# Kateridge/TransMF_AD

Hardware: AMD Instinct MI355X
Metric: volume-pairs/sec fwd+bwd(+Adam), 96^3 MRI+PET batch=8 per GPU (higher is better)
Workload: dtype f32

## Files before the change

transmf_ad_amd/csrc/conv1_gram.hip:

```cpp
#include "tmf_common.h"

namespace {

constexpr int GT_D = 8, GT_H = 8, GT_W = 32;
constexpr int GP_D = GT_D + 2, GP_H = GT_H + 4, GP_W = GT_W + 4;
constexpr int GTHR = 512, GWG = 256, NACC = 64;

__host__ __device__ constexpr int kidx(int dd, int dh, int dw) {
    return dd == 0 ? (dh == 0 ? dw : 3 + (dh - 1) * 5 + (dw + 2)) : 13 + ((dd - 1) * 5 + (dh + 2)) * 5 + (dw + 2);
}
static_assert(kidx(2, 2, 2) == 62, "63 offsets");

typedef double f64x2 __attribute__((ext_vector_type(2)));
__device__ __forceinline__ float rbf16(float v) { return __builtin_bit_cast(float, tmf_pack_bf16(v, 0.f) << 16); }

__global__ __launch_bounds__(GTHR) void c1_gram_kernel(const float* __restrict__ x, double* __restrict__ part,
                                                        int D, int H, int W, int tilesD, int tilesH, int tilesW, int ntiles, int round16) {
    constexpr int NT = GP_D * GP_H * GP_W, NS = NT > 8 * GTHR ? NT : 8 * GTHR;
    __shared__ __attribute__((aligned(16))) double smem[NS];
    double* tile = smem;
    double* red = smem;
    const int tid = threadIdx.x;
    const int g = tid & 7, hh = (tid >> 3) & 7, dd0 = tid >> 6;
    double acc[63];
// ... 62 lines not shown
    }
    const int lane = tid & 63, kq = tid >> 6;
#pragma unroll
    for (int c = 0; c < 8; ++c) {
        __syncthreads();
#pragma unroll
        for (int q = 0; q < 8; ++q) {
            const int k = c * 8 + q;
            red[q * GTHR + tid] = k < 63 ? acc[k < 63 ? k : 0] : ssum;
        }
        __syncthreads();
        double s = 0.0;
#pragma unroll
        for (int m = 0; m < 8; ++m) s += red[kq * GTHR + m * 64 + lane];
#pragma unroll
        for (int o = 32; o > 0; o >>= 1) s += __shfl_xor(s, o);
        if (lane == 0) part[(size_t)blockIdx.x * NACC + c * 8 + kq] = s;
    }
}

constexpr int GMAXC = 64;

constexpr int NGRAM = 760;
constexpr int HWG = 64, HTHR = 256, HNB = 288, HPART = 96;
constexpr int HNE = (HNB * 9 + HTHR - 1) / HTHR;

__host__ __device__ constexpr int class_tap(int cls, int j) {
    const int ax = cls >> 1, fixed = (cls & 1) ? 0 : 2, a = j / 3, b = j % 3;
    return ax == 0 ? fixed * 9 + a * 3 + b : (ax == 1 ? a * 9 + fixed * 3 + b : a * 9 + b * 3 + fixed);
}

__global__ __launch_bounds__(HTHR) void c1_shell_gram_kernel(const float* __restrict__ x, double* __restrict__ part, int B, int D, int H, int W,
                                                              int round16) {
    __shared__ double xs[HNB * 9];
    __shared__ int vbase[HNB], vcrd[HNB];
    __shared__ double red[3 * 81];
    const int tid = threadIdx.x, cls = blockIdx.y, ax = cls >> 1, side = cls & 1;
    const int n1 = ax == 0 ? H + 2 : D, n2 = ax == 2 ? H : W + 2;
    const int per = n1 * n2, total = B * per;
    const int p = tid % 81, slice = tid / 81, pi = p / 9, pj = p % 9;
    int cv_[HNE], cdd[HNE], cdh[HNE], cdw[HNE];
#pragma unroll
    for (int k = 0; k < HNE; ++k) {
        const int e = tid + k * HTHR, vi = e / 9, j = e - vi * 9, tap = class_tap(cls, j);
        cv_[k] = e < HNB * 9 ? vi : -1;
        cdd[k] = tap / 9 - 2; cdh[k] = (tap / 3) % 3 - 2; cdw[k] = tap % 3 - 2;
    }
    double acc = 0.0, eacc = 0.0;
    for (int base = blockIdx.x * HNB; base < total; base += gridDim.x * HNB) {
        __syncthreads();
        for (int vt = tid; vt < HNB; vt += HTHR) {
            const int s_ = base + vt;
            int c = -1, off = 0;
            if (s_ < total) {
                const int b = s_ / per, q = s_ - b * per, q1 = q / n2, q2 = q - q1 * n2;
                int vd, vh, vw;
                if (ax == 0) { vd = side ? D : -1; vh = q1 - 1; vw = q2 - 1; }
                else if (ax == 1) { vh = side ? H : -1; vd = q1; vw = q2 - 1; }
                else { vw = side ? W : -1; vd = q1; vh = q2; }
                c = (vd + 1) | (vh + 1) << 10 | (vw + 1) << 20;
                off = b * D * H * W;
            }
            vcrd[vt] = c; vbase[vt] = off;
        }
        __syncthreads();
#pragma unroll
        for (int k = 0; k < HNE; ++k) {
            if (cv_[k] < 0) continue;
            const int c = vcrd[cv_[k]];
            float v = 0.f;
            if (c >= 0) {
                const int ud = (c & 1023) + cdd[k], uh = ((c >> 10) & 1023) + cdh[k], uw = (c >> 20) + cdw[k];
                if (ud >= 0 && ud < D && uh >= 0 && uh < H && uw >= 0 && uw < W) v = x[(size_t)vbase[cv_[k]] + ((size_t)ud * H + uh) * W + uw];
            }
            xs[tid + k * HTHR] = (double)(round16 ? rbf16(v) : v);
        }
        __syncthreads();
        if (slice < 3) {
#pragma unroll 8
            for (int vi = slice * (HNB / 3); vi < (slice + 1) * (HNB / 3); ++vi) {
                const double xa = xs[vi * 9 + pi];
                acc = fma(xa, xs[vi * 9 + pj], acc);
                eacc += pj == 0 ? xa : 0.0;
            }
        }
    }
    __shared__ double rede[3 * 9];
    __syncthreads();
    if (slice < 3) {
        red[slice * 81 + p] = acc;
        if (pj == 0) rede[slice * 9 + pi] = eacc;
    }
    __syncthreads();
    double* row = part + ((size_t)cls * gridDim.x + blockIdx.x) * HPART;
    if (tid < 81) row[tid] = (red[tid] + red[81 + tid]) + red[162 + tid];
    else if (tid < 90) row[tid] = (rede[tid - 81] + rede[9 + tid - 81]) + rede[18 + tid - 81];
}

__global__ __launch_bounds__(1024) void c1_gram2_finish_kernel(const float* __restrict__ w, const double* __restrict__ rpart, int ngram,
                                                                const double* __restrict__ hpart, int nh, double* __restrict__ gram,
                                                                float* __restrict__ out, int C, int round16) {
    __shared__ double ra[16 * NACC];
    __shared__ double R[NACC];
    __shared__ double Hc[6 * HPART];
    __shared__ double G[27 * 27 + 27];
    __shared__ float wsh[27 * GMAXC];
    __shared__ double rows[27 * GMAXC];
    const int tid = threadIdx.x;
    {
        const int k = tid & 63, rg = tid >> 6;
        double s = 0.0;
#pragma unroll 8
        for (int i = rg; i < ngram; i += 16) s += rpart[(size_t)i * NACC + k];
        ra[rg * NACC + k] = s;
    }
    for (int e = tid; e < 27 * C; e += 1024) wsh[e] = round16 ? rbf16(w[e]) : w[e];
    for (int e = tid; e < 6 * HPART; e += 1024) {
        const int cls = e / HPART, k = e - cls * HPART;
        double s0 = 0.0, s1_ = 0.0, s2_ = 0.0, s3 = 0.0;
// ... 155 lines not shown
```

transmf_ad_amd/csrc/conv3d_mfma.hip:

```cpp
#include <type_traits>
#include "tmf_device.h"

#ifndef TMF_CONV_ACC
#define TMF_CONV_ACC 1
#endif
#ifndef TMF_CONV_BUF
#define TMF_CONV_BUF 1
#endif

namespace {

template <int KS_, int CINC_, int MT_, int NT_, int WM_, int WN_, int TD_, int TH_, int TW_, int TPS_>
struct FwdCfg {
    static constexpr int KS = KS_, CINC = CINC_, MT = MT_, NT = NT_, WM = WM_, WN = WN_;
    static constexpr int TD = TD_, TH = TH_, TW = TW_, TPS = TPS_;
    static constexpr int PAD = KS / 2;
    static constexpr int HD = TD + 2 * PAD, HH = TH + 2 * PAD, HW = TW + 2 * PAD;
    static constexpr int NHALO = HD * HH * HW;
    static constexpr int CP = CINC + 4;
    static constexpr int NPOS = TD * TH * TW;
    static constexpr int NB = 32 * NT * WN;
    static constexpr int NTAPS = KS * KS * KS;
    static constexpr int NSTAGES = NTAPS / TPS;
    static constexpr int BSTAGE = TPS * CINC * NB;
// ... 1111 lines not shown
        else mma_bricks(std::integral_constant<int, 3>{});
    }

#pragma unroll
    for (int t = 0; t < C::TPW; ++t) {
        const int tap0 = C::PACK ? 2 * (wave + 8 * t) : tap_base + t;
        if (t < tap_cnt && tap0 < 27) {
#pragma unroll
            for (int j = 0; j < C::NT; ++j) {
                const int co = co0 + j * 32 + l31;
#pragma unroll
                for (int r = 0; r < 16; ++r) {
                    const int m = (r & 3) + 8 * (r >> 2) + 4 * hsel;
                    const int tap = C::PACK ? tap0 + (r >> 3) : tap0;
                    const int ci = ci0 + (C::PACK ? (m & 15) : m);
                    if (tap < 27 && ci < Cin && co < Cout)
                        partial[(((size_t)split * 27 + tap) * Cin + ci) * Cout + co] = acc[t][j][r];
                }
            }
        }
    }
}

template <int NT>
__global__ __launch_bounds__(256) void conv1x1_wgrad_kernel(
    const float* __restrict__ x, const float* __restrict__ dz, float* __restrict__ partial,
    long npos, int Cin, int Cout, int slabs_per_block) {
    const int tid = threadIdx.x;
    const int lane = tid & 63;
    const int wave = __builtin_amdgcn_readfirstlane(tid >> 6);
    const int l31 = lane & 31, hsel = lane >> 5;
    const int ci = blockIdx.y * 32 + l31;
    const int co0 = blockIdx.z * 32 * NT;
    f32x16 acc[NT];
#pragma unroll
    for (int j = 0; j < NT; ++j)
#pragma unroll
        for (int r = 0; r < 16; ++r) acc[j][r] = 0.f;
    const long p_begin = ((long)blockIdx.x * slabs_per_block) * 256 + wave * 64;
    for (int sl = 0; sl < slabs_per_block; ++sl) {
        const long pb = p_begin + (long)sl * 256;
#pragma unroll 8
        for (int q = 0; q < 32; ++q) {
            const long p = pb + 2 * q + hsel;
            const bool pv = p < npos;
            const float av = (pv && ci < Cin) ? x[p * Cin + ci] : 0.f;
#pragma unroll
            for (int j = 0; j < NT; ++j) {
                const int co = co0 + j * 32 + l31;
                const float bv = (pv && co < Cout) ? dz[p * Cout + co] : 0.f;
                acc[j] = __builtin_amdgcn_mfma_f32_32x32x2f32(av, bv, acc[j], 0, 0, 0);
            }
        }
    }
    const int split = blockIdx.x * 4 + wave;
#pragma unroll
    for (int j = 0; j < NT; ++j) {
        const int co = co0 + j * 32 + l31;
#pragma unroll
        for (int r = 0; r < 16; ++r) {
            const int cr = blockIdx.y * 32 + (r & 3) + 8 * (r >> 2) + 4 * hsel;
            if (cr < Cin && co < Cout) partial[((size_t)split * Cin + cr) * Cout + co] = acc[j][r];
        }
    }
}

struct WgPlan {
    int nt, tilesD, tilesH, tilesW, ntiles, tps, nsplit, gy, gz;
    int small;
    int pack;
};

WgPlan plan_wgrad(int B, int D, int H, int W, int cin, int cout) {
    WgPlan p;
    const int mind = D < H ? (D < W ? D : W) : (H < W ? H : W);
    p.small = !(mind >= 16 || (long)D * H * W >= 4096);
    const int td = 4, th = p.small ? 4 : 8, tw = p.small ? 4 : 8;
    const bool w8 = (cin % 4 == 0) && (cout % 4 == 0) && conv_waves() >= 8;
    p.nt = (cout <= 32 || w8) ? 1 : 2;
    p.tilesD = tmf_cdiv(D, td); p.tilesH = tmf_cdiv(H, th); p.tilesW = tmf_cdiv(W, tw);
    p.ntiles = B * p.tilesD * p.tilesH * p.tilesW;
    p.pack = w8 && cin <= 16;
    p.gy = p.pack ? 1 : tmf_cdiv(cin, 32);
    p.gz = tmf_cdiv(cout, 32 * p.nt);
    const int groups = p.gy * p.gz;
    int want = 256 / groups;
    if (want < 1) want = 1;
    if (want > p.ntiles) want = p.ntiles;
    p.tps = tmf_cdiv(p.ntiles, want);
    p.nsplit = tmf_cdiv(p.ntiles, p.tps);
    return p;
}

struct Wg1Plan { int nt, gy, gz, spb, nblk, nsplit; };
Wg1Plan plan_wgrad1(long npos, int cin, int cout) {
    Wg1Plan p;
    p.nt = cout <= 32 ? 1 : 2;
    p.gy = tmf_cdiv(cin, 32);
    p.gz = tmf_cdiv(cout, 32 * p.nt);
    const long slabs = (npos + 255) / 256;
    int want = 1024 / (p.gy * p.gz);
    if (want < 1) want = 1;
    if (want > slabs) want = (int)slabs;
    p.spb = (int)((slabs + want - 1) / want);
    p.nblk = (int)((slabs + p.spb - 1) / p.spb);
    p.nsplit = p.nblk * 4;
    return p;
}

constexpr int C1_TD = 4, C1_TH = 8, C1_TW = 8;
constexpr int C1_HD = C1_TD + 2, C1_HH = C1_TH + 2, C1_HW = C1_TW + 2;
constexpr int C1_NHALO = C1_HD * C1_HH * C1_HW;

__device__ __forceinline__ constexpr int c1_tapoff(int tap) {
    return tap >= 27 ? 0 : ((tap / 9) * C1_HH + (tap / 3) % 3) * C1_HW + tap % 3;
}

__global__ __launch_bounds__(256) void conv3d_c1_fwd_kernel(
    const float* __restrict__ x, const float* __restrict__ w, float* __restrict__ z,
    float* __restrict__ stat_partial, int D, int H, int W, int Cout,
    int tilesD, int tilesH, int tilesW, int ntiles) {
    __shared__ float halo[C1_NHALO];
    __shared__ float red[4 * 32 * 2];
    const int tid = threadIdx.x;
    const int lane = tid & 63;
    const int wave = __builtin_amdgcn_readfirstlane(tid >> 6);
    const int l31 = lane & 31, hsel = lane >> 5;
    const int tile = xcd_contiguous(blockIdx.x, ntiles);
    int t = tile;
// ... 282 lines not shown
        using S1w8p = WgCfg<1, 4, 4, 4, 8, 16>;
        const bool w8 = vec && conv_waves() >= 8;
        if (w8 && p.pack) {
            if (!p.small) TMF_WG_LAUNCH(L1w8p, true);
            else          TMF_WG_LAUNCH(S1w8p, true);
        } else if (w8) {
            if (!p.small && p.nt == 1) TMF_WG_LAUNCH(L1w8, true);
            else if (!p.small)         TMF_WG_LAUNCH(L2w8, true);
            else if (p.nt == 1)        TMF_WG_LAUNCH(S1w8, true);
            else                       TMF_WG_LAUNCH(S2w8, true);
        }
        else if (!p.small && p.nt == 1) { if (vec) TMF_WG_LAUNCH(L1, true); else TMF_WG_LAUNCH(L1, false); }
        else if (!p.small)         { if (vec) TMF_WG_LAUNCH(L2, true); else TMF_WG_LAUNCH(L2, false); }
        else if (p.nt == 1)        { if (vec) TMF_WG_LAUNCH(S1, true); else TMF_WG_LAUNCH(S1, false); }
        else                       { if (vec) TMF_WG_LAUNCH(S2, true); else TMF_WG_LAUNCH(S2, false); }
#undef TMF_WG_LAUNCH
        if ((rc = tmf_launch_result("tmf_conv3d_wgrad"))) return rc;
        nelem = 27L * cin * cout;
        nsplit = p.nsplit;
    } else {
        const long npos = (long)B * D * H * W;
        const Wg1Plan p = plan_wgrad1(npos, cin, cout);
        dim3 grid(p.nblk, p.gy, p.gz), block(256);
        if (p.nt == 1) hipLaunchKernelGGL(conv1x1_wgrad_kernel<1>, grid, block, 0, s, x, dz, partial, npos, cin, cout, p.spb);
        else           hipLaunchKernelGGL(conv1x1_wgrad_kernel<2>, grid, block, 0, s, x, dz, partial, npos, cin, cout, p.spb);
        if ((rc = tmf_launch_result("tmf_conv3d_wgrad(1x1)"))) return rc;
        nelem = (long)cin * cout;
        nsplit = p.nsplit;
    }
    return tmf_reduce_slabs(partial, nsplit, nelem, partial + (size_t)nsplit * nelem, dw, s, "tmf_conv3d_wgrad(reduce)",
                            dw_layout == TMF_DW_REFERENCE ? cin : 0, cout);
}

extern "C" int tmf_conv3d_c1_stat_blocks(int B, int D, int H, int W, int cout) {
    if (B <= 0 || D <= 0 || H <= 0 || W <= 0 || cout <= 0) return 0;
    return plan_c1(B, D, H, W, cout).ntiles;
}

extern "C" int tmf_conv3d_c1_fwd(const float* x, const float* w, float* z, float* stat_partial,
                                 int B, int D, int H, int W, int cout, void* stream) {
    TMF_REQUIRE_PTR(x); TMF_REQUIRE_PTR(w); TMF_REQUIRE_PTR(z);
    TMF_REQUIRE(B > 0 && D > 0 && H > 0 && W > 0 && cout > 0, TMF_E_SHAPE, "tmf_conv3d_c1_fwd: non-positive dimension");
    TMF_REQUIRE((long)D * H * W * cout < (1L << 31), TMF_E_SHAPE, "tmf_conv3d_c1_fwd: one sample exceeds 2^31 elements");
    const C1Plan p = plan_c1(B, D, H, W, cout);
    hipLaunchKernelGGL(conv3d_c1_fwd_kernel, dim3(p.ntiles, p.nby), dim3(256), 0, (hipStream_t)stream,
                       x, w, z, stat_partial, D, H, W, cout, p.tilesD, p.tilesH, p.tilesW, p.ntiles);
    return tmf_launch_result("tmf_conv3d_c1_fwd");
}
// ... 30 lines not shown
```

transmf_ad_amd/csrc/tmf_device.h:

```cpp
#pragma once
#include "tmf_common.h"

typedef float f32x2 __attribute__((ext_vector_type(2)));
typedef int i32x4 __attribute__((ext_vector_type(4)));

__device__ __forceinline__ i32x4 make_rsrc(const void* p, unsigned bytes) {
    const unsigned long long a = (unsigned long long)p;
    return i32x4{(int)(unsigned)a, (int)((unsigned)(a >> 32) & 0xFFFFu), (int)bytes, 0x00020000};
}
__device__ __forceinline__ void blds16(int voff, i32x4 rsrc, int soff, unsigned lds_wave_base) {
    asm volatile("s_mov_b32 m0, %3\n\ts_nop 0\n\tbuffer_load_dwordx4 %0, %1, %2 offen lds" ::"v"(voff), "s"(rsrc), "s"(soff), "s"(lds_wave_base) : "memory");
}
__device__ __forceinline__ void blds16_uniform(int voff, i32x4 rsrc, int soff, unsigned lds_wave_base) {
    asm volatile("" : "+s"(soff));
    rsrc = i32x4{__builtin_amdgcn_readfirstlane(rsrc[0]), __builtin_amdgcn_readfirstlane(rsrc[1]), __builtin_amdgcn_readfirstlane(rsrc[2]),
                 __builtin_amdgcn_readfirstlane(rsrc[3])};
    asm volatile("s_mov_b32 m0, %3\n\ts_nop 0\n\tbuffer_load_dwordx4 %0, %1, %2 offen lds" ::"v"(voff), "s"(rsrc), "s"(soff), "s"(lds_wave_base) : "memory");
}
template <typename V> __device__ __forceinline__ void bload16(V& dst, int voff, i32x4 rsrc, int soff) {
    asm volatile("buffer_load_dwordx4 %0, %1, %2, %3 offen" : "=v"(dst) : "v"(voff), "s"(rsrc), "s"(soff) : "memory");
}
template <typename V> __device__ __forceinline__ void bload16_pinned(V& dst, int voff, i32x4 rsrc, int soff) {
    asm volatile("" : "+s"(soff));
    asm volatile("buffer_load_dwordx4 %0, %1, %2, %3 offen" : "=v"(dst) : "v"(voff), "s"(rsrc), "s"(soff) : "memory");
}
template <int N> __device__ __forceinline__ void vm_wait() { asm volatile("s_waitcnt vmcnt(%0)" ::"n"(N) : "memory"); }

__device__ __forceinline__ void store_guard() {
    __builtin_amdgcn_sched_barrier(0);
    asm volatile("s_nop 0");
    __builtin_amdgcn_sched_barrier(0);
}

__device__ __forceinline__ int frag_row(int r, int hsel) { return (r & 3) + 8 * (r >> 2) + 4 * hsel; }

__device__ __forceinline__ float gelu_f(float h) { return 0.5f * h * (1.f + erff(h * 0.70710678118654752f)); }
__device__ __forceinline__ float gelu_grad_f(float h) {
    return 0.5f * (1.f + erff(h * 0.70710678118654752f)) + h * 0.3989422804014327f * expf(-0.5f * h * h);
}
__device__ __forceinline__ float half_sum(float v) {
    v += __shfl_xor(v, 16); v += __shfl_xor(v, 8); v += __shfl_xor(v, 4); v += __shfl_xor(v, 2); v += __shfl_xor(v, 1);
    return v;
}

__device__ __forceinline__ void split3_trunc(float x, float& h, float& m, float& l) {
    h = __builtin_bit_cast(float, __builtin_bit_cast(unsigned, x) & 0xFFFF0000u);
    const float r = x - h;
    m = __builtin_bit_cast(float, __builtin_bit_cast(unsigned, r) & 0xFFFF0000u);
    l = r - m;
}
__device__ __forceinline__ unsigned short bf16_bits_rne(float a) { return __builtin_bit_cast(unsigned short, (__bf16)a); }
__device__ __forceinline__ void split3_rne(float a, unsigned short& h, unsigned short& m, unsigned short& l) {
    h = bf16_bits_rne(a);
    const float r1 = a - __builtin_bit_cast(float, (unsigned)h << 16);
    m = bf16_bits_rne(r1);
    const float r2 = r1 - __builtin_bit_cast(float, (unsigned)m << 16);
    l = bf16_bits_rne(r2);
}
```

transmf_ad_amd/csrc/token_gemm.hip:

```cpp
#include <type_traits>
#include "tmf_device.h"

namespace {

constexpr int TM = 16, TTHR = 256;

struct TokArgs {
    const float* A; const float* W; float* Y;
    int R, K, N;
    const float* ln_g; const float* ln_b; float eps; float* ln_mean; float* ln_rstd; float* ln_out;
    const float* bias; const float* res; float* pre;
    const float* gelu_h;
    const float* lnb_x; const float* lnb_mean; const float* lnb_rstd; const float* lnb_g;
    const float* add1; const float* add2;
    float* lnb_partial; float* colsum_partial; int partial_stride;
    const float* mask; float* Y2;
};

__device__ __forceinline__ float hsum(f32x4 v) { return v[0] + v[1] + v[2] + v[3]; }
__device__ __forceinline__ float hsum(f32x2 v) { return v[0] + v[1]; }
__device__ __forceinline__ f32x4 minus(f32x4 v, float mu) { return f32x4{v[0] - mu, v[1] - mu, v[2] - mu, v[3] - mu}; }
__device__ __forceinline__ f32x2 minus(f32x2 v, float mu) { return f32x2{v[0] - mu, v[1] - mu}; }
__device__ __forceinline__ float sumsq(f32x4 d) { return d[0] * d[0] + d[1] * d[1] + d[2] * d[2] + d[3] * d[3]; }
__device__ __forceinline__ float sumsq(f32x2 d) { return d[0] * d[0] + d[1] * d[1]; }
// ... 357 lines not shown
                                         float* ln_mean, float* ln_rstd, float* ln_out, float* gelu_pre, const float* mask,
                                         void* stream) {
    TMF_REQUIRE_PTR(x); TMF_REQUIRE_PTR(w); TMF_REQUIRE_PTR(y); TMF_REQUIRE_PTR(mask);
    return tmf_tok_linear_fwd_impl(x, w, bias, residual, y, R, K, Nout, ln_gamma, ln_beta, eps, ln_mean, ln_rstd, ln_out, gelu_pre,
                                   mask, stream);
}

extern "C" int tmf_tok_linear_bwd_input_masked(const float* dy, const float* w, float* dx, int R, int Nout, int K,
                                               const float* gelu_pre, const float* ln_x, const float* ln_mean,
                                               const float* ln_rstd, const float* ln_gamma, const float* add1,
                                               const float* add2, float* ln_partial, float* bias_partial,
                                               int partial_stride, const float* mask, float* dx_masked, void* stream) {
    TMF_REQUIRE_PTR(dy); TMF_REQUIRE_PTR(w); TMF_REQUIRE_PTR(dx); TMF_REQUIRE_PTR(mask);
    return tmf_tok_linear_bwd_input_impl(dy, w, dx, R, Nout, K, gelu_pre, ln_x, ln_mean, ln_rstd, ln_gamma, add1, add2, ln_partial,
                                         bias_partial, partial_stride, mask, dx_masked, stream);
}

namespace {

constexpr int WG_MAXP = 32, WG_NSPLIT = 8;
struct WgMulti {
    const float* dy[WG_MAXP]; const float* x[WG_MAXP]; float* dw[WG_MAXP];
    int R[WG_MAXP], N[WG_MAXP], K[WG_MAXP], tile0[WG_MAXP + 1], elem0[WG_MAXP + 1];
    int nprob;
};

__global__ __launch_bounds__(256, 2) void tok_wgrad_multi_kernel(const WgMulti p, float* __restrict__ partial, long total_elems) {
    __shared__ float red[3][32 * 32];
    const int tid = threadIdx.x, lane = tid & 63;
    const int wave = __builtin_amdgcn_readfirstlane(tid >> 6);
    const int l31 = lane & 31, hsel = lane >> 5;
    int q = 0;
    while (q + 1 < p.nprob && (int)blockIdx.x >= p.tile0[q + 1]) ++q;
    const int t = blockIdx.x - p.tile0[q];
    const int tiles_k = p.K[q] >> 5;
    const int n0 = (t / tiles_k) * 32, k0 = (t % tiles_k) * 32;
    const int R = p.R[q], N = p.N[q], K = p.K[q];
    int rows = (R + WG_NSPLIT - 1) / WG_NSPLIT;
    rows = (rows + 7) & ~7;
    const int rb = blockIdx.y * rows + wave * (rows >> 2);
    const float* dy = p.dy[q] + n0 + l31;
    const float* xx = p.x[q] + k0 + l31;
    f32x16 acc;
#pragma unroll
    for (int r = 0; r < 16; ++r) acc[r] = 0.f;
    const int steps = rows >> 3;
    constexpr int UB = 16;
    for (int s0 = 0; s0 < steps; s0 += UB) {
        float a[UB], b[UB];
#pragma unroll
        for (int u = 0; u < UB; ++u) {
            const int row = rb + 2 * (s0 + u) + hsel;
            const bool ok = (s0 + u) < steps && row < R;
            const int rr = ok ? row : 0;
            a[u] = dy[(size_t)rr * N];
            b[u] = xx[(size_t)rr * K];
            a[u] = ok ? a[u] : 0.f;
        }
#pragma unroll
        for (int u = 0; u < UB; ++u) acc = __builtin_amdgcn_mfma_f32_32x32x2f32(a[u], b[u], acc, 0, 0, 0);
    }
    if (wave > 0) {
#pragma unroll
        for (int r = 0; r < 16; ++r) red[wave - 1][((r & 3) + 8 * (r >> 2) + 4 * hsel) * 32 + l31] = acc[r];
    }
    __syncthreads();
    if (wave == 0) {
        float* dst = partial + (size_t)blockIdx.y * total_elems + p.elem0[q];
#pragma unroll
        for (int r = 0; r < 16; ++r) {
            const int i = (r & 3) + 8 * (r >> 2) + 4 * hsel;
            const float v = acc[r] + red[0][i * 32 + l31] + red[1][i * 32 + l31] + red[2][i * 32 + l31];
            dst[(size_t)(n0 + i) * K + k0 + l31] = v;
        }
    }
}

__global__ __launch_bounds__(256) void tok_wgrad_multi_reduce_kernel(const WgMulti p, const float* __restrict__ partial,
                                                                     long total_elems) {
    const long e = (long)blockIdx.x * 256 + threadIdx.x;
    if (e >= total_elems) return;
    float s = 0.f;
#pragma unroll
    for (int k = 0; k < WG_NSPLIT; ++k) s += partial[(size_t)k * total_elems + e];
    int q = 0;
    while (q + 1 < p.nprob && e >= p.elem0[q + 1]) ++q;
    p.dw[q][e - p.elem0[q]] = s;
}

int fill_multi(WgMulti& m, int nprob, const float* const* dy, const float* const* x, float* const* dw,
               const int* R, const int* N, const int* K, const char* fn) {
    TMF_REQUIRE(nprob > 0 && nprob <= WG_MAXP, TMF_E_SHAPE, "%s: 1..%d problems, got %d", fn, WG_MAXP, nprob);
    m.nprob = nprob;
    m.tile0[0] = 0; m.elem0[0] = 0;
    for (int q = 0; q < nprob; ++q) {
        TMF_REQUIRE(R[q] > 0 && N[q] > 0 && K[q] > 0 && N[q] % 32 == 0 && K[q] % 32 == 0, TMF_E_SHAPE,
                    "%s: problem %d: R=%d N=%d K=%d (N and K must be multiples of 32)", fn, q, R[q], N[q], K[q]);
        m.R[q] = R[q]; m.N[q] = N[q]; m.K[q] = K[q];
        if (dy) { m.dy[q] = dy[q]; m.x[q] = x[q]; m.dw[q] = dw[q]; }
        m.tile0[q + 1] = m.tile0[q] + (N[q] / 32) * (K[q] / 32);
        m.elem0[q + 1] = m.elem0[q] + N[q] * K[q];
    }
    return TMF_OK;
}

}

extern "C" size_t tmf_tok_wgrad_multi_workspace_bytes(int nprob, const int* N, const int* K) {
    if (nprob <= 0 || nprob > WG_MAXP || N == nullptr || K == nullptr) return 0;
    size_t e = 0;
    for (int q = 0; q < nprob; ++q) e += (size_t)N[q] * K[q];
    return e * WG_NSPLIT * 4;
}

extern "C" int tmf_tok_wgrad_multi(int nprob, const float* const* dy, const float* const* x, float* const* dw,
                                   const int* R, const int* N, const int* K, void* workspace, size_t workspace_bytes,
                                   void* stream) {
    TMF_REQUIRE_PTR(dy); TMF_REQUIRE_PTR(x); TMF_REQUIRE_PTR(dw); TMF_REQUIRE_PTR(R); TMF_REQUIRE_PTR(N); TMF_REQUIRE_PTR(K);
    TMF_REQUIRE_PTR(workspace);
    WgMulti m = {};
    int rc = fill_multi(m, nprob, dy, x, dw, R, N, K, "tmf_tok_wgrad_multi");
    if (rc) return rc;
    for (int q = 0; q < nprob; ++q) { TMF_REQUIRE_PTR(dy[q]); TMF_REQUIRE_PTR(x[q]); TMF_REQUIRE_PTR(dw[q]); }
    const size_t need = tmf_tok_wgrad_multi_workspace_bytes(nprob, N, K);
    TMF_REQUIRE(workspace_bytes >= need, TMF_E_WORKSPACE, "tmf_tok_wgrad_multi: workspace %zu B < required %zu B",
                workspace_bytes, need);
    const long total = m.elem0[nprob];
    hipStream_t s = (hipStream_t)stream;
    hipLaunchKernelGGL(tok_wgrad_multi_kernel, dim3(m.tile0[nprob], WG_NSPLIT), dim3(256), 0, s, m, (float*)workspace, total);
    if ((rc = tmf_launch_result("tmf_tok_wgrad_multi"))) return rc;
    hipLaunchKernelGGL(tok_wgrad_multi_reduce_kernel, dim3((unsigned)tmf_cdiv(total, 256L)), dim3(256), 0, s, m,
                       (const float*)workspace, total);
    return tmf_launch_result("tmf_tok_wgrad_multi(reduce)");
}
```

transmf_ad_amd/csrc/token_ops.hip:

```cpp
#include "tmf_device.h"

static thread_local char g_err[512] = "";

void tmf_set_error(const char* fmt, ...) {
    va_list ap;
    va_start(ap, fmt);
    vsnprintf(g_err, sizeof g_err, fmt, ap);
    va_end(ap);
}

extern "C" int tmf_version(void) { return 1; }
extern "C" const char* tmf_last_error_string(void) { return g_err; }

namespace {

constexpr int LN_MAXV = 8;

template <int VEC>
__global__ __launch_bounds__(256) void layernorm_fwd_kernel(
    const float* __restrict__ x, const float* __restrict__ gamma, const float* __restrict__ beta,
    const float* __restrict__ residual, float* __restrict__ y, float* __restrict__ mean, float* __restrict__ rstd,
    int rows, int dim, float eps) {
    const int lane = threadIdx.x & 63;
    const int row = blockIdx.x * 4 + (threadIdx.x >> 6);
// ... 83 lines not shown
                red[(wave * 2 + 0) * dim + i + q] = ag[u * VEC + q];
                red[(wave * 2 + 1) * dim + i + q] = ab[u * VEC + q];
            }
        }
    }
    __syncthreads();
    for (int e = threadIdx.x; e < 2 * dim; e += 256) {
        const float a = red[e] + red[2 * dim + e] + red[4 * dim + e] + red[6 * dim + e];
        partial[(size_t)blockIdx.x * 2 * dim + e] = a;
    }
}

__global__ __launch_bounds__(256) void mask_mul_kernel(const float* __restrict__ x, const float* __restrict__ mask,
                                                       float* __restrict__ y, long n) {
    const long i = ((long)blockIdx.x * 256 + threadIdx.x) * 4;
    if (i + 4 <= n) {
        const f32x4 a = *reinterpret_cast<const f32x4*>(x + i), m = *reinterpret_cast<const f32x4*>(mask + i);
        *reinterpret_cast<f32x4*>(y + i) = f32x4{a[0] * m[0], a[1] * m[1], a[2] * m[2], a[3] * m[3]};
    } else {
        for (long j = i; j < n; ++j) y[j] = x[j] * mask[j];
    }
}

__global__ __launch_bounds__(256) void token_pool_fwd_kernel(const float* __restrict__ mri, const float* __restrict__ pet,
                                                             float* __restrict__ cls, int32_t* __restrict__ argmax,
                                                             int B, int N, int dim) {
    __shared__ float ssum[4][64], smax[4][64];
    __shared__ int sarg[4][64];
    const int cgroups = (dim + 63) / 64;
    const int cg = blockIdx.x % cgroups, mod = (blockIdx.x / cgroups) % 2, b = blockIdx.x / (2 * cgroups);
    const int cl = threadIdx.x & 63, tl = threadIdx.x >> 6;
    const int c = cg * 64 + cl;
    float s = 0.f, mx = -INFINITY;
    int am = 0;
    if (c < dim) {
        const float* src = (mod == 0 ? mri : pet) + (size_t)b * N * dim + c;
        for (int n = tl; n < N; n += 4) {
            const float v = src[(size_t)n * dim];
            s += v;
            if (v > mx || v != v) { mx = v; am = n; }
        }
    }
    ssum[tl][cl] = s; smax[tl][cl] = mx; sarg[tl][cl] = am;
    __syncthreads();
    if (tl == 0 && c < dim) {
#pragma unroll
        for (int k = 1; k < 4; ++k) {
            s += ssum[k][cl];
            const float v = smax[k][cl];
            const int a = sarg[k][cl];
            if (v != v) {
                if (mx == mx || a > am) { mx = v; am = a; }
            } else if (mx == mx && (v > mx || (v == mx && a < am))) { mx = v; am = a; }
        }
        cls[(size_t)b * 4 * dim + mod * dim + c] = s / N;
        cls[(size_t)b * 4 * dim + (2 + mod) * dim + c] = mx;
        argmax[((size_t)b * 2 + mod) * dim + c] = am;
    }
}

__global__ void token_pool_bwd_kernel(const float* __restrict__ dcls, const int32_t* __restrict__ argmax,
                                      float* __restrict__ dmri, float* __restrict__ dpet, int B, int N, int dim) {
    const long i = (long)blockIdx.x * blockDim.x + threadIdx.x;
    const long total = (long)B * 2 * N * dim;
    if (i >= total) return;
    const int c = i % dim;
    const int n = (i / dim) % N;
    const int mod = (i / ((long)dim * N)) % 2;
    const int b = i / ((long)dim * N * 2);
    const float gavg = dcls[(size_t)b * 4 * dim + mod * dim + c];
// ... 182 lines not shown
    return tmf_layernorm_bwd_impl(x, gamma, mean, rstd, dy, dx, partial, rows, dim, nullptr, nullptr, stream);
}

extern "C" int tmf_layernorm_bwd_masked(const float* x, const float* gamma, const float* mean, const float* rstd,
                                        const float* dy, float* dx, float* partial, int rows, int dim,
                                        const float* mask, float* dx_masked, void* stream) {
    TMF_REQUIRE_PTR(x); TMF_REQUIRE_PTR(gamma); TMF_REQUIRE_PTR(mean); TMF_REQUIRE_PTR(rstd);
    TMF_REQUIRE_PTR(dy); TMF_REQUIRE_PTR(dx); TMF_REQUIRE_PTR(partial); TMF_REQUIRE_PTR(mask);
    return tmf_layernorm_bwd_impl(x, gamma, mean, rstd, dy, dx, partial, rows, dim, mask, dx_masked, stream);
}

extern "C" int tmf_mask_mul(const float* x, const float* mask, float* y, long n, void* stream) {
    TMF_REQUIRE_PTR(x); TMF_REQUIRE_PTR(mask); TMF_REQUIRE_PTR(y);
    TMF_REQUIRE_ALIGNED(x); TMF_REQUIRE_ALIGNED(mask); TMF_REQUIRE_ALIGNED(y);
    TMF_REQUIRE(n > 0 && n < (1L << 40), TMF_E_SHAPE, "tmf_mask_mul: n=%ld", n);
    hipLaunchKernelGGL(mask_mul_kernel, dim3((unsigned)tmf_cdiv(n, 1024L)), dim3(256), 0, (hipStream_t)stream, x, mask, y, n);
    return tmf_launch_result("tmf_mask_mul");
}

extern "C" int tmf_token_pool_fwd(const float* mri, const float* pet, float* cls, int32_t* argmax,
                                  int B, int N, int dim, void* stream) {
    TMF_REQUIRE_PTR(mri); TMF_REQUIRE_PTR(pet); TMF_REQUIRE_PTR(cls); TMF_REQUIRE_PTR(argmax);
    TMF_REQUIRE(B > 0 && N > 0 && dim > 0, TMF_E_SHAPE, "tmf_token_pool_fwd: B=%d N=%d dim=%d", B, N, dim);
    hipLaunchKernelGGL(token_pool_fwd_kernel, dim3(B * 2 * tmf_cdiv(dim, 64)), dim3(256), 0, (hipStream_t)stream,
                       mri, pet, cls, argmax, B, N, dim);
    return tmf_launch_result("tmf_token_pool_fwd");
}

extern "C" int tmf_token_pool_bwd(const float* dcls, const int32_t* argmax, float* dmri, float* dpet,
                                  int B, int N, int dim, void* stream) {
    TMF_REQUIRE_PTR(dcls); TMF_REQUIRE_PTR(argmax); TMF_REQUIRE_PTR(dmri); TMF_REQUIRE_PTR(dpet);
    TMF_REQUIRE(B > 0 && N > 0 && dim > 0, TMF_E_SHAPE, "tmf_token_pool_bwd: B=%d N=%d dim=%d", B, N, dim);
    const long total = (long)B * 2 * N * dim;
    hipLaunchKernelGGL(token_pool_bwd_kernel, dim3(tmf_cdiv(total, 256)), dim3(256), 0, (hipStream_t)stream,
                       dcls, argmax, dmri, dpet, B, N, dim);
    return tmf_launch_result("tmf_token_pool_bwd");
}
```

Baseline: 995.8.

## Share LDS-staged TN GEMM tile for weight grads; widen shell gram and token pool

Adds a shared LDS-staged, register-prefetched TN GEMM tile helper with 64x64*NT tiles and optional float4 loads. Both the 1x1 conv weight-gradient kernel and the token weight-gradient multi kernel now use it. The token path picks its split count with a cost model and skips the reduce kernel when the split is 1. The shell gram kernel runs three sub-groups per block and stages values in LDS as floats instead of doubles, and token pooling uses 16 lanes per column with unrolled loads. These target poor global load coalescing and occupancy, at the cost of more LDS per block and a different reduction order.

```diff
diff --git a/transmf_ad_amd/csrc/conv1_gram.hip b/transmf_ad_amd/csrc/conv1_gram.hip
--- a/transmf_ad_amd/csrc/conv1_gram.hip
+++ b/transmf_ad_amd/csrc/conv1_gram.hip
@@ -108,8 +108,8 @@
 constexpr int GMAXC = 64;
 
 constexpr int NGRAM = 760;
-constexpr int HWG = 64, HTHR = 256, HNB = 288, HPART = 96;
-constexpr int HNE = (HNB * 9 + HTHR - 1) / HTHR;
+constexpr int HWG = 64, HSG = 3, HSUB = 256, HTHR = HSG * HSUB, HNB = 288, HPART = 96;
+constexpr int HNE = (HNB * 9 + HSUB - 1) / HSUB;
 
 __host__ __device__ constexpr int class_tap(int cls, int j) {
     const int ax = cls >> 1, fixed = (cls & 1) ? 0 : 2, a = j / 3, b = j % 3;
@@ -118,24 +118,28 @@
 
 __global__ __launch_bounds__(HTHR) void c1_shell_gram_kernel(const float* __restrict__ x, double* __restrict__ part, int B, int D, int H, int W,
                                                               int round16) {
-    __shared__ double xs[HNB * 9];
-    __shared__ int vbase[HNB], vcrd[HNB];
-    __shared__ double red[3 * 81];
-    const int tid = threadIdx.x, cls = blockIdx.y, ax = cls >> 1, side = cls & 1;
+    __shared__ float xs_[HSG][HNB * 9];
+    __shared__ int vbase_[HSG][HNB], vcrd_[HSG][HNB];
+    __shared__ double red[HSG * 3 * 81];
+    const int sg = threadIdx.x / HSUB, tid = threadIdx.x % HSUB;
+    float* xs = xs_[sg];
+    int *vbase = vbase_[sg], *vcrd = vcrd_[sg];
+    const int cls = blockIdx.y, ax = cls >> 1, side = cls & 1;
     const int n1 = ax == 0 ? H + 2 : D, n2 = ax == 2 ? H : W + 2;
     const int per = n1 * n2, total = B * per;
     const int p = tid % 81, slice = tid / 81, pi = p / 9, pj = p % 9;
     int cv_[HNE], cdd[HNE], cdh[HNE], cdw[HNE];
 #pragma unroll
     for (int k = 0; k < HNE; ++k) {
-        const int e = tid + k * HTHR, vi = e / 9, j = e - vi * 9, tap = class_tap(cls, j);
+        const int e = tid + k * HSUB, vi = e / 9, j = e - vi * 9, tap = class_tap(cls, j);
         cv_[k] = e < HNB * 9 ? vi : -1;
         cdd[k] = tap / 9 - 2; cdh[k] = (tap / 3) % 3 - 2; cdw[k] = tap % 3 - 2;
     }
     double acc = 0.0, eacc = 0.0;
-    for (int base = blockIdx.x * HNB; base < total; base += gridDim.x * HNB) {
-        __syncthreads();
-        for (int vt = tid; vt < HNB; vt += HTHR) {
+    for (int base0 = blockIdx.x * HSG * HNB; base0 < total; base0 += gridDim.x * HSG * HNB) {
+        const int base = base0 + sg * HNB;
+        __syncthreads();
+        for (int vt = tid; vt < HNB; vt += HSUB) {
             const int s_ = base + vt;
             int c = -1, off = 0;
             if (s_ < total) {
@@ -159,28 +163,33 @@
                 const int ud = (c & 1023) + cdd[k], uh = ((c >> 10) & 1023) + cdh[k], uw = (c >> 20) + cdw[k];
                 if (ud >= 0 && ud < D && uh >= 0 && uh < H && uw >= 0 && uw < W) v = x[(size_t)vbase[cv_[k]] + ((size_t)ud * H + uh) * W + uw];
             }
-            xs[tid + k * HTHR] = (double)(round16 ? rbf16(v) : v);
+            xs[tid + k * HSUB] = round16 ? rbf16(v) : v;
         }
         __syncthreads();
         if (slice < 3) {
 #pragma unroll 8
             for (int vi = slice * (HNB / 3); vi < (slice + 1) * (HNB / 3); ++vi) {
-                const double xa = xs[vi * 9 + pi];
-                acc = fma(xa, xs[vi * 9 + pj], acc);
+                const double xa = (double)xs[vi * 9 + pi];
+                acc = fma(xa, (double)xs[vi * 9 + pj], acc);
                 eacc += pj == 0 ? xa : 0.0;
             }
         }
     }
-    __shared__ double rede[3 * 9];
+    __shared__ double rede[HSG * 3 * 9];
     __syncthreads();
     if (slice < 3) {
-        red[slice * 81 + p] = acc;
-        if (pj == 0) rede[slice * 9 + pi] = eacc;
+        red[(sg * 3 + slice) * 81 + p] = acc;
+        if (pj == 0) rede[(sg * 3 + slice) * 9 + pi] = eacc;
     }
     __syncthreads();
     double* row = part + ((size_t)cls * gridDim.x + blockIdx.x) * HPART;
-    if (tid < 81) row[tid] = (red[tid] + red[81 + tid]) + red[162 + tid];
-    else if (tid < 90) row[tid] = (rede[tid - 81] + rede[9 + tid - 81]) + rede[18 + tid - 81];
+    if (threadIdx.x < 90) {
+        const int t = threadIdx.x;
+        double s_ = 0.0;
+#pragma unroll
+        for (int q = 0; q < HSG * 3; ++q) s_ += t < 81 ? red[q * 81 + t] : rede[q * 9 + t - 81];
+        row[t] = s_;
+    }
 }
 
 __global__ __launch_bounds__(1024) void c1_gram2_finish_kernel(const float* __restrict__ w, const double* __restrict__ rpart, int ngram,
diff --git a/transmf_ad_amd/csrc/conv3d_mfma.hip b/transmf_ad_amd/csrc/conv3d_mfma.hip
--- a/transmf_ad_amd/csrc/conv3d_mfma.hip
+++ b/transmf_ad_amd/csrc/conv3d_mfma.hip
@@ -1157,47 +1157,16 @@
     }
 }
 
-template <int NT>
+template <int NT, bool VEC>
 __global__ __launch_bounds__(256) void conv1x1_wgrad_kernel(
     const float* __restrict__ x, const float* __restrict__ dz, float* __restrict__ partial,
-    long npos, int Cin, int Cout, int slabs_per_block) {
-    const int tid = threadIdx.x;
-    const int lane = tid & 63;
-    const int wave = __builtin_amdgcn_readfirstlane(tid >> 6);
-    const int l31 = lane & 31, hsel = lane >> 5;
-    const int ci = blockIdx.y * 32 + l31;
-    const int co0 = blockIdx.z * 32 * NT;
-    f32x16 acc[NT];
-#pragma unroll
-    for (int j = 0; j < NT; ++j)
-#pragma unroll
-        for (int r = 0; r < 16; ++r) acc[j][r] = 0.f;
-    const long p_begin = ((long)blockIdx.x * slabs_per_block) * 256 + wave * 64;
-    for (int sl = 0; sl < slabs_per_block; ++sl) {
-        const long pb = p_begin + (long)sl * 256;
-#pragma unroll 8
-        for (int q = 0; q < 32; ++q) {
-            const long p = pb + 2 * q + hsel;
-            const bool pv = p < npos;
-            const float av = (pv && ci < Cin) ? x[p * Cin + ci] : 0.f;
-#pragma unroll
-            for (int j = 0; j < NT; ++j) {
-                const int co = co0 + j * 32 + l31;
-                const float bv = (pv && co < Cout) ? dz[p * Cout + co] : 0.f;
-                acc[j] = __builtin_amdgcn_mfma_f32_32x32x2f32(av, bv, acc[j], 0, 0, 0);
-            }
-        }
-    }
-    const int split = blockIdx.x * 4 + wave;
-#pragma unroll
-    for (int j = 0; j < NT; ++j) {
-        const int co = co0 + j * 32 + l31;
-#pragma unroll
-        for (int r = 0; r < 16; ++r) {
-            const int cr = blockIdx.y * 32 + (r & 3) + 8 * (r >> 2) + 4 * hsel;
-            if (cr < Cin && co < Cout) partial[((size_t)split * Cin + cr) * Cout + co] = acc[j][r];
-        }
-    }
+    long npos, int Cin, int Cout, int per) {
+    __shared__ float xs[TN_ROWS * 64];
+    __shared__ float ds[TN_ROWS * 64 * NT];
+    const long p0 = (long)blockIdx.x * per;
+    const long p1 = p0 + per < npos ? p0 + per : npos;
+    tn_gemm_tile<NT, VEC>(x, Cin, dz, Cout, p0, p1, blockIdx.y * 64, blockIdx.z * 64 * NT,
+                          partial + (size_t)blockIdx.x * Cin * Cout, xs, ds);
 }
 
 struct WgPlan {
@@ -1227,19 +1196,19 @@
     return p;
 }
 
-struct Wg1Plan { int nt, gy, gz, spb, nblk, nsplit; };
+struct Wg1Plan { int nt, gy, gz, per, nblk, nsplit; };
 Wg1Plan plan_wgrad1(long npos, int cin, int cout) {
     Wg1Plan p;
-    p.nt = cout <= 32 ? 1 : 2;
-    p.gy = tmf_cdiv(cin, 32);
-    p.gz = tmf_cdiv(cout, 32 * p.nt);
-    const long slabs = (npos + 255) / 256;
-    int want = 1024 / (p.gy * p.gz);
+    p.nt = cout <= 64 ? 1 : 2;
+    p.gy = tmf_cdiv(cin, 64);
+    p.gz = tmf_cdiv(cout, 64 * p.nt);
+    int want = 256 / (p.gy * p.gz);
     if (want < 1) want = 1;
-    if (want > slabs) want = (int)slabs;
-    p.spb = (int)((slabs + want - 1) / want);
-    p.nblk = (int)((slabs + p.spb - 1) / p.spb);
-    p.nsplit = p.nblk * 4;
+    long per = ((npos + want - 1) / want + 7) / 8 * 8;
+    if (per < TN_ROWS) per = TN_ROWS;
+    p.per = (int)per;
+    p.nblk = (int)((npos + per - 1) / per);
+    p.nsplit = p.nblk;
     return p;
 }
 
@@ -1568,8 +1537,9 @@
         const long npos = (long)B * D * H * W;
         const Wg1Plan p = plan_wgrad1(npos, cin, cout);
         dim3 grid(p.nblk, p.gy, p.gz), block(256);
-        if (p.nt == 1) hipLaunchKernelGGL(conv1x1_wgrad_kernel<1>, grid, block, 0, s, x, dz, partial, npos, cin, cout, p.spb);
-        else           hipLaunchKernelGGL(conv1x1_wgrad_kernel<2>, grid, block, 0, s, x, dz, partial, npos, cin, cout, p.spb);
+        auto k = p.nt == 1 ? (vec ? conv1x1_wgrad_kernel<1, true> : conv1x1_wgrad_kernel<1, false>)
+                           : (vec ? conv1x1_wgrad_kernel<2, true> : conv1x1_wgrad_kernel<2, false>);
+        hipLaunchKernelGGL(k, grid, block, 0, s, x, dz, partial, npos, cin, cout, p.per);
         if ((rc = tmf_launch_result("tmf_conv3d_wgrad(1x1)"))) return rc;
         nelem = (long)cin * cout;
         nsplit = p.nsplit;
diff --git a/transmf_ad_amd/csrc/tmf_device.h b/transmf_ad_amd/csrc/tmf_device.h
--- a/transmf_ad_amd/csrc/tmf_device.h
+++ b/transmf_ad_amd/csrc/tmf_device.h
@@ -43,6 +43,98 @@
     return v;
 }
 
+constexpr int TN_ROWS = 64;
+
+template <bool VEC>
+__device__ __forceinline__ f32x4 tn_fetch4(const float* __restrict__ src, long r, long r_end, int C, int c) {
+    f32x4 v = {0.f, 0.f, 0.f, 0.f};
+    if (r < r_end) {
+        const float* q = src + r * C + c;
+        if (VEC) {
+            if (c < C) v = *reinterpret_cast<const f32x4*>(q);
+        } else {
+#pragma unroll
+            for (int j = 0; j < 4; ++j)
+                if (c + j < C) v[j] = q[j];
+        }
+    }
+    return v;
+}
+
+template <int NT, bool VEC>
+__device__ __forceinline__ void tn_gemm_tile(const float* __restrict__ A, int M, const float* __restrict__ B, int N, long r0, long r1,
+                                             int i0, int j0, float* __restrict__ out, float* as, float* bs) {
+    constexpr int TN = 64 * NT;
+    constexpr int AV = TN_ROWS * 64 / 4 / 256;
+    constexpr int BV = TN_ROWS * TN / 4 / 256;
+    const int tid = threadIdx.x;
+    const int lane = tid & 63;
+    const int wave = __builtin_amdgcn_readfirstlane(tid >> 6);
+    const int l31 = lane & 31, hsel = lane >> 5;
+    const int mt = wave & 1, nh = wave >> 1;
+    const int it = i0 + mt * 32, jt = j0 + nh * 32 * NT;
+    const bool active = it < M && jt < N;
+    f32x16 acc[NT];
+#pragma unroll
+    for (int j = 0; j < NT; ++j)
+#pragma unroll
+        for (int r = 0; r < 16; ++r) acc[j][r] = 0.f;
+    f32x4 ar[AV], br[BV];
+    auto fetch = [&](long rb) {
+#pragma unroll
+        for (int q = 0; q < AV; ++q) {
+            const int e = tid + q * 256;
+            ar[q] = tn_fetch4<VEC>(A, rb + (e >> 4), r1, M, i0 + (e & 15) * 4);
+        }
+#pragma unroll
+        for (int q = 0; q < BV; ++q) {
+            const int e = tid + q * 256;
+            br[q] = tn_fetch4<VEC>(B, rb + e / (TN / 4), r1, N, j0 + (e % (TN / 4)) * 4);
+        }
+    };
+    fetch(r0);
+    const float* ap = as + hsel * 64 + mt * 32 + l31;
+    const float* bp = bs + hsel * TN + nh * 32 * NT + l31;
+    for (long rb = r0; rb < r1; rb += TN_ROWS) {
+        __syncthreads();
+#pragma unroll
+        for (int q = 0; q < AV; ++q) *reinterpret_cast<f32x4*>(&as[(tid + q * 256) * 4]) = ar[q];
+#pragma unroll
+        for (int q = 0; q < BV; ++q) *reinterpret_cast<f32x4*>(&bs[(tid + q * 256) * 4]) = br[q];
+        __syncthreads();
+        if (rb + TN_ROWS < r1) fetch(rb + TN_ROWS);
+        const long rem = r1 - rb;
+        const int kgroups = rem >= TN_ROWS ? TN_ROWS / 16 : (int)((rem + 15) >> 4);
+        if (active) {
+            for (int g = 0; g < kgroups; ++g) {
+                float av[8], bv[NT][8];
+#pragma unroll
+                for (int u = 0; u < 8; ++u) {
+                    av[u] = ap[(g * 8 + u) * 2 * 64];
+#pragma unroll
+                    for (int j = 0; j < NT; ++j) bv[j][u] = bp[(g * 8 + u) * 2 * TN + j * 32];
+                }
+                __builtin_amdgcn_sched_barrier(0);
+#pragma unroll
+                for (int u = 0; u < 8; ++u)
+#pragma unroll
+                    for (int j = 0; j < NT; ++j)
+                        acc[j] = __builtin_amdgcn_mfma_f32_32x32x2f32(av[u], bv[j][u], acc[j], 0, 0, 0);
+            }
+        }
+    }
+    if (!active) return;
+#pragma unroll
+    for (int j = 0; j < NT; ++j) {
+        const int col = jt + j * 32 + l31;
+#pragma unroll
+        for (int r = 0; r < 16; ++r) {
+            const int row = it + frag_row(r, hsel);
+            if (row < M && col < N) out[(size_t)row * N + col] = acc[j][r];
+        }
+    }
+}
+
 __device__ __forceinline__ void split3_trunc(float x, float& h, float& m, float& l) {
     h = __builtin_bit_cast(float, __builtin_bit_cast(unsigned, x) & 0xFFFF0000u);
     const float r = x - h;
diff --git a/transmf_ad_amd/csrc/token_gemm.hip b/transmf_ad_amd/csrc/token_gemm.hip
--- a/transmf_ad_amd/csrc/token_gemm.hip
+++ b/transmf_ad_amd/csrc/token_gemm.hip
@@ -403,70 +403,59 @@
 struct WgMulti {
     const float* dy[WG_MAXP]; const float* x[WG_MAXP]; float* dw[WG_MAXP];
     int R[WG_MAXP], N[WG_MAXP], K[WG_MAXP], tile0[WG_MAXP + 1], elem0[WG_MAXP + 1];
-    int nprob;
+    int nprob, nsplit;
 };
 
-__global__ __launch_bounds__(256, 2) void tok_wgrad_multi_kernel(const WgMulti p, float* __restrict__ partial, long total_elems) {
-    __shared__ float red[3][32 * 32];
-    const int tid = threadIdx.x, lane = tid & 63;
-    const int wave = __builtin_amdgcn_readfirstlane(tid >> 6);
-    const int l31 = lane & 31, hsel = lane >> 5;
+template <int NT, bool VEC>
+__global__ __launch_bounds__(256) void tok_wgrad_multi_kernel(const WgMulti p, float* __restrict__ partial, long total_elems) {
+    __shared__ float as[TN_ROWS * 64];
+    __shared__ float bs[TN_ROWS * 64 * NT];
+    const int bx = xcd_contiguous(blockIdx.x, gridDim.x);
     int q = 0;
-    while (q + 1 < p.nprob && (int)blockIdx.x >= p.tile0[q + 1]) ++q;
-    const int t = blockIdx.x - p.tile0[q];
-    const int tiles_k = p.K[q] >> 5;
-    const int n0 = (t / tiles_k) * 32, k0 = (t % tiles_k) * 32;
+    while (q + 1 < p.nprob && bx >= p.tile0[q + 1]) ++q;
+    const int t = bx - p.tile0[q];
     const int R = p.R[q], N = p.N[q], K = p.K[q];
-    int rows = (R + WG_NSPLIT - 1) / WG_NSPLIT;
+    const int tiles_k = (K + 64 * NT - 1) / (64 * NT);
+    int rows = (R + p.nsplit - 1) / p.nsplit;
     rows = (rows + 7) & ~7;
-    const int rb = blockIdx.y * rows + wave * (rows >> 2);
-    const float* dy = p.dy[q] + n0 + l31;
-    const float* xx = p.x[q] + k0 + l31;
-    f32x16 acc;
-#pragma unroll
-    for (int r = 0; r < 16; ++r) acc[r] = 0.f;
-    const int steps = rows >> 3;
-    constexpr int UB = 16;
-    for (int s0 = 0; s0 < steps; s0 += UB) {
-        float a[UB], b[UB];
-#pragma unroll
-        for (int u = 0; u < UB; ++u) {
-            const int row = rb + 2 * (s0 + u) + hsel;
-            const bool ok = (s0 + u) < steps && row < R;
-            const int rr = ok ? row : 0;
-            a[u] = dy[(size_t)rr * N];
-            b[u] = xx[(size_t)rr * K];
-            a[u] = ok ? a[u] : 0.f;
-        }
-#pragma unroll
-        for (int u = 0; u < UB; ++u) acc = __builtin_amdgcn_mfma_f32_32x32x2f32(a[u], b[u], acc, 0, 0, 0);
-    }
-    if (wave > 0) {
-#pragma unroll
-        for (int r = 0; r < 16; ++r) red[wave - 1][((r & 3) + 8 * (r >> 2) + 4 * hsel) * 32 + l31] = acc[r];
-    }
-    __syncthreads();
-    if (wave == 0) {
-        float* dst = partial + (size_t)blockIdx.y * total_elems + p.elem0[q];
-#pragma unroll
-        for (int r = 0; r < 16; ++r) {
-            const int i = (r & 3) + 8 * (r >> 2) + 4 * hsel;
-            const float v = acc[r] + red[0][i * 32 + l31] + red[1][i * 32 + l31] + red[2][i * 32 + l31];
-            dst[(size_t)(n0 + i) * K + k0 + l31] = v;
-        }
-    }
-}
-
+    int r0 = blockIdx.y * rows;
+    if (r0 > R) r0 = R;
+    const int r1 = r0 + rows < R ? r0 + rows : R;
+    float* out = p.nsplit == 1 ? p.dw[q] : partial + (size_t)blockIdx.y * total_elems + p.elem0[q];
+    tn_gemm_tile<NT, VEC>(p.dy[q], N, p.x[q], K, r0, r1, (t / tiles_k) * 64, (t % tiles_k) * 64 * NT, out, as, bs);
+}
+
+template <bool VEC>
 __global__ __launch_bounds__(256) void tok_wgrad_multi_reduce_kernel(const WgMulti p, const float* __restrict__ partial,
                                                                      long total_elems) {
-    const long e = (long)blockIdx.x * 256 + threadIdx.x;
+    constexpr int V = VEC ? 4 : 1;
+    const long e = ((long)blockIdx.x * 256 + threadIdx.x) * V;
     if (e >= total_elems) return;
-    float s = 0.f;
-#pragma unroll
-    for (int k = 0; k < WG_NSPLIT; ++k) s += partial[(size_t)k * total_elems + e];
     int q = 0;
     while (q + 1 < p.nprob && e >= p.elem0[q + 1]) ++q;
-    p.dw[q][e - p.elem0[q]] = s;
+    if (VEC) {
+        f32x4 s = *reinterpret_cast<const f32x4*>(partial + e);
+        for (int k = 1; k < p.nsplit; ++k) {
+            const f32x4 v = *reinterpret_cast<const f32x4*>(partial + (size_t)k * total_elems + e);
+            s[0] += v[0]; s[1] += v[1]; s[2] += v[2]; s[3] += v[3];
+        }
+        *reinterpret_cast<f32x4*>(p.dw[q] + (e - p.elem0[q])) = s;
+    } else {
+        float s = partial[e];
+        for (int k = 1; k < p.nsplit; ++k) s += partial[(size_t)k * total_elems + e];
+        p.dw[q][e - p.elem0[q]] = s;
+    }
+}
+
+int wg_pick_nsplit(int tiles, int rmax, long total_elems) {
+    int best_n = 1;
+    long best = -1;
+    for (int n = 1; n <= WG_NSPLIT; ++n) {
+        const int rows = ((rmax + n - 1) / n + 7) & ~7;
+        const long cost = (long)tmf_cdiv((long)tiles * n, 256) * rows + (n > 1 ? n * total_elems / 10000 : 0);
+        if (best < 0 || cost < best) { best = cost; best_n = n; }
+    }
+    return best_n;
 }
 
 int fill_multi(WgMulti& m, int nprob, const float* const* dy, const float* const* x, float* const* dw,
@@ -474,12 +463,15 @@
     TMF_REQUIRE(nprob > 0 && nprob <= WG_MAXP, TMF_E_SHAPE, "%s: 1..%d problems, got %d", fn, WG_MAXP, nprob);
     m.nprob = nprob;
     m.tile0[0] = 0; m.elem0[0] = 0;
+    int kmax = 0;
+    for (int q = 0; q < nprob; ++q) kmax = K[q] > kmax ? K[q] : kmax;
+    const int tn = kmax <= 64 ? 64 : 128;
     for (int q = 0; q < nprob; ++q) {
         TMF_REQUIRE(R[q] > 0 && N[q] > 0 && K[q] > 0 && N[q] % 32 == 0 && K[q] % 32 == 0, TMF_E_SHAPE,
                     "%s: problem %d: R=%d N=%d K=%d (N and K must be multiples of 32)", fn, q, R[q], N[q], K[q]);
         m.R[q] = R[q]; m.N[q] = N[q]; m.K[q] = K[q];
         if (dy) { m.dy[q] = dy[q]; m.x[q] = x[q]; m.dw[q] = dw[q]; }
-        m.tile0[q + 1] = m.tile0[q] + (N[q] / 32) * (K[q] / 32);
+        m.tile0[q + 1] = m.tile0[q] + tmf_cdiv(N[q], 64) * tmf_cdiv(K[q], tn);
         m.elem0[q + 1] = m.elem0[q] + N[q] * K[q];
     }
     return TMF_OK;
@@ -507,10 +499,22 @@
     TMF_REQUIRE(workspace_bytes >= need, TMF_E_WORKSPACE, "tmf_tok_wgrad_multi: workspace %zu B < required %zu B",
                 workspace_bytes, need);
     const long total = m.elem0[nprob];
+    int rmax = 0, kmax = 0;
+    bool vec = ((uintptr_t)workspace & 15u) == 0;
+    for (int q = 0; q < nprob; ++q) {
+        rmax = R[q] > rmax ? R[q] : rmax;
+        kmax = K[q] > kmax ? K[q] : kmax;
+        vec = vec && (((uintptr_t)dy[q] | (uintptr_t)x[q] | (uintptr_t)dw[q]) & 15u) == 0;
+    }
+    m.nsplit = wg_pick_nsplit(m.tile0[nprob], rmax, total);
     hipStream_t s = (hipStream_t)stream;
-    hipLaunchKernelGGL(tok_wgrad_multi_kernel, dim3(m.tile0[nprob], WG_NSPLIT), dim3(256), 0, s, m, (float*)workspace, total);
+    const dim3 grid(m.tile0[nprob], m.nsplit), block(256);
+    auto k = kmax <= 64 ? (vec ? tok_wgrad_multi_kernel<1, true> : tok_wgrad_multi_kernel<1, false>)
+                        : (vec ? tok_wgrad_multi_kernel<2, true> : tok_wgrad_multi_kernel<2, false>);
+    hipLaunchKernelGGL(k, grid, block, 0, s, m, (float*)workspace, total);
     if ((rc = tmf_launch_result("tmf_tok_wgrad_multi"))) return rc;
-    hipLaunchKernelGGL(tok_wgrad_multi_reduce_kernel, dim3((unsigned)tmf_cdiv(total, 256L)), dim3(256), 0, s, m,
-                       (const float*)workspace, total);
+    if (m.nsplit == 1) return TMF_OK;
+    auto kr = vec ? tok_wgrad_multi_reduce_kernel<true> : tok_wgrad_multi_reduce_kernel<false>;
+    hipLaunchKernelGGL(kr, dim3((unsigned)tmf_cdiv(total, vec ? 1024L : 256L)), block, 0, s, m, (const float*)workspace, total);
     return tmf_launch_result("tmf_tok_wgrad_multi(reduce)");
 }
diff --git a/transmf_ad_amd/csrc/token_ops.hip b/transmf_ad_amd/csrc/token_ops.hip
--- a/transmf_ad_amd/csrc/token_ops.hip
+++ b/transmf_ad_amd/csrc/token_ops.hip
@@ -129,11 +129,12 @@
     }
 }
 
-__global__ __launch_bounds__(256) void token_pool_fwd_kernel(const float* __restrict__ mri, const float* __restrict__ pet,
-                                                             float* __restrict__ cls, int32_t* __restrict__ argmax,
-                                                             int B, int N, int dim) {
-    __shared__ float ssum[4][64], smax[4][64];
-    __shared__ int sarg[4][64];
+constexpr int TP_LANES = 16;
+__global__ __launch_bounds__(64 * TP_LANES) void token_pool_fwd_kernel(const float* __restrict__ mri, const float* __restrict__ pet,
+                                                                       float* __restrict__ cls, int32_t* __restrict__ argmax,
+                                                                       int B, int N, int dim) {
+    __shared__ float ssum[TP_LANES][64], smax[TP_LANES][64];
+    __shared__ int sarg[TP_LANES][64];
     const int cgroups = (dim + 63) / 64;
     const int cg = blockIdx.x % cgroups, mod = (blockIdx.x / cgroups) % 2, b = blockIdx.x / (2 * cgroups);
     const int cl = threadIdx.x & 63, tl = threadIdx.x >> 6;
@@ -142,17 +143,25 @@
     int am = 0;
     if (c < dim) {
         const float* src = (mod == 0 ? mri : pet) + (size_t)b * N * dim + c;
-        for (int n = tl; n < N; n += 4) {
-            const float v = src[(size_t)n * dim];
+        auto take = [&](float v, int n) {
             s += v;
             if (v > mx || v != v) { mx = v; am = n; }
-        }
+        };
+        int n = tl;
+        for (; n + 3 * TP_LANES < N; n += 4 * TP_LANES) {
+            float v[4];
+#pragma unroll
+            for (int u = 0; u < 4; ++u) v[u] = src[(size_t)(n + u * TP_LANES) * dim];
+#pragma unroll
+            for (int u = 0; u < 4; ++u) take(v[u], n + u * TP_LANES);
+        }
+        for (; n < N; n += TP_LANES) take(src[(size_t)n * dim], n);
     }
     ssum[tl][cl] = s; smax[tl][cl] = mx; sarg[tl][cl] = am;
     __syncthreads();
     if (tl == 0 && c < dim) {
 #pragma unroll
-        for (int k = 1; k < 4; ++k) {
+        for (int k = 1; k < TP_LANES; ++k) {
             s += ssum[k][cl];
             const float v = smax[k][cl];
             const int a = sarg[k][cl];
@@ -381,7 +390,7 @@
                                   int B, int N, int dim, void* stream) {
     TMF_REQUIRE_PTR(mri); TMF_REQUIRE_PTR(pet); TMF_REQUIRE_PTR(cls); TMF_REQUIRE_PTR(argmax);
     TMF_REQUIRE(B > 0 && N > 0 && dim > 0, TMF_E_SHAPE, "tmf_token_pool_fwd: B=%d N=%d dim=%d", B, N, dim);
-    hipLaunchKernelGGL(token_pool_fwd_kernel, dim3(B * 2 * tmf_cdiv(dim, 64)), dim3(256), 0, (hipStream_t)stream,
+    hipLaunchKernelGGL(token_pool_fwd_kernel, dim3(B * 2 * tmf_cdiv(dim, 64)), dim3(64 * TP_LANES), 0, (hipStream_t)stream,
                        mri, pet, cls, argmax, B, N, dim);
     return tmf_launch_result("tmf_token_pool_fwd");
 }
```

New measurement: 994.4, median of 5. Within noise of the previous version (-0.1%).
